# consensus-shipyard/ipc-filecoin-proofs

Measured on AMD Instinct MI355X. Metric: Merkle proofs verified/sec + HBM GB/s, 1M-receipt synthetic tipset, 1/2/4/8 GPU, higher is better.
Workload: dtype u64; 1 GPU; BASELINE.json configs[2] (the 1M-receipt tipset the metric is quoted on): 1000000 receipts (Amtv0<Receipt> + one Amt<...; receipts_per_gpu=1000000, claims_per_gpu=1000000, witness_blocks_per_gpu=1288038, witness_bytes_per_gpu=439923915, scan_matches=1002, device=AMD Radeon Graphics

## Files before the change

ipc-filecoin-proofs_amd/csrc/common.h:

```cpp
#pragma once
#include <hip/hip_runtime.h>

#include <cstdint>
#include <cstdio>
#include <memory>
#include <cstring>
#include <string>
#include <utility>
#include <vector>

#include "ipcfp.h"
#include "kernels/event_table.h"

namespace ipcfp {

struct DevPool {
    std::vector<std::pair<void*, size_t>> free_;
    size_t cached_bytes = 0;
    hipError_t take(void** out, size_t bytes, size_t* cap);
    void give(void* p, size_t cap);
    void drain();
    ~DevPool() { drain(); }
};
extern thread_local DevPool* g_tls_pool;
// ... 20 lines not shown
#endif
#ifndef IPCFP_PARSE_RESIDENT_DEFAULT
#define IPCFP_PARSE_RESIDENT_DEFAULT 1
#endif

struct ipcfp_ctx {
    int device = -1;
    hipStream_t stream = nullptr;
    hipStream_t stream_k1 = nullptr;
    hipStream_t stream_aux = nullptr;
    ipcfp::ScanParams scan_hint{};
    bool has_scan_hint = false;
    hipEvent_t aux_event = nullptr;
    std::string last_error;
    hipDeviceProp_t props{};
    ipcfp::DevPool pool;
    bool profiling = false;
    int profile_only = -1;
    std::vector<ipcfp::ProfiledLaunch> launches;
    std::vector<hipEvent_t> free_events;
    uint64_t prof_count[IPCFP_K_COUNT] = {};
    double prof_ms[IPCFP_K_COUNT] = {};
    uint8_t* pinned = nullptr;
    size_t pinned_cap = 0, pinned_used = 0;
    struct PendingRead {
        void* dst;
        size_t off, n;
        hipStream_t stream;
        bool hold = false;
    };
    std::vector<PendingRead> pending;
    int call_depth = 0;
    uint8_t* ctl_dev = nullptr;
    uint8_t* ctl_host = nullptr;
    uint32_t ctl_used_zero = 0, ctl_used_ff = 0;
    bool ctl_primed = false;
    bool ctl_preprimed = false;
    struct CtlRead {
        void* dst;
        uint32_t off, n;
    };
    std::vector<CtlRead> ctl_reads;
    hipEvent_t join_event = nullptr;
    hipEvent_t spin_event = nullptr;
    bool spin_sync = true;
    ipcfp::UploadRing* upload_ring = nullptr;
    hipStream_t stream_copy = nullptr;
    ipcfp::UploadTask* upload_task = nullptr;
    struct ClaimsExpand {
        bool pending = false;
        const void* compact_d = nullptr;
        const ipcfp_event_claim_group_t* groups_d = nullptr;
        uint32_t n = 0, n_groups = 0;
        const uint8_t* cblob_d = nullptr;
        uint64_t cblob_len = 0, cap_blob = 0;
        void* claims_out_d = nullptr;
        uint8_t* blob_out_d = nullptr;
        uint32_t* scratch_u32 = nullptr;
        uint64_t* scan_scratch = nullptr;
    } claims_expand;
    struct ClaimsRebase {
        bool pending = false;
        void* claims_d = nullptr;
        uint32_t n = 0;
        uint64_t base = 0, blob_len = 0;
        uint64_t full_len = 0;
// ... 23 lines not shown
    void* hamt_etabs = nullptr;
    size_t hamt_etabs_bytes = 0;
};

namespace ipcfp {

int set_error(ipcfp_ctx* ctx, int rc, const char* fmt, ...);

#define IPCFP_HIP(ctx, call)                                                                    \
    do {                                                                                        \
        hipError_t _e = (call);                                                                 \
        if (_e != hipSuccess)                                                                   \
            return ::ipcfp::set_error((ctx), IPCFP_E_HIP, "%s failed: %s (%s:%d)", #call,       \
                                      hipGetErrorString(_e), __FILE__, __LINE__);               \
    } while (0)

constexpr uint32_t kCtlHalf = 2048;

inline void* ctl_take(ipcfp_ctx* ctx, uint32_t bytes, bool ff) {
    if (!ctx->ctl_dev) return nullptr;
    bytes = (bytes + 7u) & ~7u;
    uint32_t& used = ff ? ctx->ctl_used_ff : ctx->ctl_used_zero;
    if (used + bytes > kCtlHalf) return nullptr;
    if (!ctx->ctl_primed) {
        if (hipMemcpyAsync(ctx->ctl_dev, ctx->ctl_host, 2 * kCtlHalf, hipMemcpyHostToDevice, ctx->stream) != hipSuccess) return nullptr;
        ctx->ctl_primed = true;
    }
    void* p = ctx->ctl_dev + (ff ? kCtlHalf : 0u) + used;
    used += bytes;
    ctx->ctl_preprimed = false;
    return p;
}
inline void ctl_preprime(ipcfp_ctx* ctx) {
    if (!ctx->ctl_dev || ctx->ctl_preprimed || ctx->call_depth != 1) return;
    if (hipMemcpyAsync(ctx->ctl_dev, ctx->ctl_host, 2 * kCtlHalf, hipMemcpyHostToDevice, ctx->stream) == hipSuccess) {
        ctx->ctl_preprimed = true;
    }
}
inline hipError_t ctl_fetch(ipcfp_ctx* ctx) {
    if (!ctx->ctl_dev || !ctx->ctl_primed) return hipSuccess;
    return hipMemcpyAsync(ctx->ctl_host + 2 * kCtlHalf, ctx->ctl_dev, 2 * kCtlHalf, hipMemcpyDeviceToHost, ctx->stream);
}
inline bool ctl_owns(const ipcfp_ctx* ctx, const void* dev_ptr) {
    const uint8_t* p = static_cast<const uint8_t*>(dev_ptr);
    return ctx->ctl_dev && p >= ctx->ctl_dev && p < ctx->ctl_dev + 2 * kCtlHalf;
}
template <typename T>
inline T ctl_value(const ipcfp_ctx* ctx, const void* dev_ptr) {
    T v;
    std::memcpy(&v, ctx->ctl_host + 2 * kCtlHalf + (static_cast<const uint8_t*>(dev_ptr) - ctx->ctl_dev), sizeof(T));
    return v;
}

inline hipError_t d2h_small(ipcfp_ctx* ctx, void* dst, const void* src_d, size_t n, hipStream_t s) {
    const size_t need = (n + 15) & ~size_t(15);
    if (!ctx->pinned || ctx->pinned_used + need > ctx->pinned_cap) return hipMemcpyAsync(dst, src_d, n, hipMemcpyDeviceToHost, s);
    const size_t off = ctx->pinned_used;
    ctx->pinned_used += need;
    ctx->pending.push_back({dst, off, n, s, false});
    return hipMemcpyAsync(ctx->pinned + off, src_d, n, hipMemcpyDeviceToHost, s);
}
inline hipError_t h2d_small(ipcfp_ctx* ctx, void* dst_d, const void* src, size_t n, hipStream_t s) {
    const size_t need = (n + 15) & ~size_t(15);
    if (!ctx->pinned || ctx->pinned_used + need > ctx->pinned_cap) return hipMemcpyAsync(dst_d, src, n, hipMemcpyHostToDevice, s);
    const size_t off = ctx->pinned_used;
    ctx->pinned_used += need;
    std::memcpy(ctx->pinned + off, src, n);
    ctx->pending.push_back({nullptr, off, 0, s, true});
    return hipMemcpyAsync(dst_d, ctx->pinned + off, n, hipMemcpyHostToDevice, s);
}
hipError_t wait_stream(ipcfp_ctx* ctx, hipStream_t s);

inline hipError_t sync_stream(ipcfp_ctx* ctx, hipStream_t s, bool last_of_call = false) {
    const bool ctl = s == ctx->stream && !ctx->ctl_reads.empty();
    if (ctl) (void)ctl_fetch(ctx);
    if (last_of_call && s == ctx->stream && ctx->ctl_dev && ctx->ctl_primed && !ctx->ctl_preprimed && ctx->call_depth == 1 &&
        hipMemcpyAsync(ctx->ctl_dev, ctx->ctl_host, 2 * kCtlHalf, hipMemcpyHostToDevice, ctx->stream) == hipSuccess) {
        ctx->ctl_preprimed = true;
    }
    const hipError_t e = wait_stream(ctx, s);
    if (ctl) {
        if (e == hipSuccess)
            for (auto& r : ctx->ctl_reads) std::memcpy(r.dst, ctx->ctl_host + 2 * kCtlHalf + r.off, r.n);
        ctx->ctl_reads.clear();
    }
    bool others = false;
    for (auto& r : ctx->pending) {
        if (r.stream == s) {
            if (r.dst && e == hipSuccess) std::memcpy(r.dst, ctx->pinned + r.off, r.n);
            r.dst = nullptr;
            r.hold = false;
        } else if (r.dst || r.hold) {
            others = true;
        }
    }
    if (!others) {
        ctx->pending.clear();
        ctx->pinned_used = 0;
    }
    return e;
}

int upload(ipcfp_ctx* ctx, void* dst_d, const void* src, size_t bytes, hipStream_t s);
bool upload_ring_mode();
UploadTask* upload_task_start(ipcfp_ctx* ctx, void* dst0, const void* src0, size_t bytes0, void* dst1, const void* src1, size_t bytes1);
int upload_task_wait(ipcfp_ctx* ctx);
int claims_ready(ipcfp_ctx* ctx);

struct ProfileScope {
// ... 58 lines not shown
        std::swap(p, o.p);
        std::swap(count, o.count);
        std::swap(cap, o.cap);
        std::swap(owner, o.owner);
    }
};

template <typename T>
inline hipError_t ctl_words(ipcfp_ctx* ctx, DevBuf<T>& own, T*& p, size_t count, bool ff) {
    p = static_cast<T*>(ctl_take(ctx, uint32_t(count * sizeof(T)), ff));
    if (p) return hipSuccess;
    hipError_t e = own.alloc(count);
    if (e != hipSuccess) return e;
    p = own.p;
    return hipMemsetAsync(own.p, ff ? 0xff : 0, count * sizeof(T), ctx->stream);
}
inline hipError_t ctl_read(ipcfp_ctx* ctx, void* dst, const void* p, size_t n) {
    if (ctl_owns(ctx, p)) {
        ctx->ctl_reads.push_back({dst, uint32_t(static_cast<const uint8_t*>(p) - ctx->ctl_dev), uint32_t(n)});
        return hipSuccess;
    }
    return d2h_small(ctx, dst, p, n, ctx->stream);
}

struct CallScope {
    DevPool* prev;
    ipcfp_ctx* ctx;
    explicit CallScope(ipcfp_ctx* c) : prev(g_tls_pool), ctx(c) {
        g_tls_pool = &c->pool;
        if (c->call_depth++ == 0) {
            c->pending.clear();
            c->pinned_used = 0;
            c->ctl_used_zero = c->ctl_used_ff = 0;
            c->ctl_primed = c->ctl_preprimed;
            c->ctl_reads.clear();
        }
    }
    ~CallScope() {
        g_tls_pool = prev;
        --ctx->call_depth;
    }
};
#define IPCFP_ENTER(ctx)                                 \
    IPCFP_HIP((ctx), hipSetDevice((ctx)->device));       \
    ::ipcfp::CallScope _ipcfp_call_scope(ctx)

inline uint32_t div_up(uint64_t a, uint64_t b) { return uint32_t((a + b - 1) / b); }

}

namespace ipcfp {
struct EnumCached {
    uint64_t root[5];
    int version = 0, vkind = 0;
    DevBuf<uint8_t> leaves;
    uint64_t n = 0;
    uint64_t error = ~0ULL;
    bool dense = false;
    uint64_t lo = 0, hi = ~0ULL;
};
struct EventTableCached {
    uint64_t root[5];
    uint64_t lo = 0, hi = ~0ULL;
    DevBuf<ReceiptRec> receipts;
    const EventRec* events = nullptr;
    uint64_t n = 0;
// ... 41 lines not shown
```

ipc-filecoin-proofs_amd/csrc/host/context.cpp:

```cpp
#include <algorithm>
#include <chrono>
#include <cstdarg>
#include <cstdlib>
#include <cstring>
#include <vector>

#include "../common.h"

namespace ipcfp {

int set_error(ipcfp_ctx* ctx, int rc, const char* fmt, ...) {
    char buf[512];
    va_list ap;
    va_start(ap, fmt);
    vsnprintf(buf, sizeof buf, fmt, ap);
    va_end(ap);
    if (ctx) ctx->last_error = buf;
    return rc;
}

thread_local DevPool* g_tls_pool = nullptr;

hipError_t wait_stream(ipcfp_ctx* ctx, hipStream_t s) {
    if (!ctx->spin_sync || !ctx->spin_event) return hipStreamSynchronize(s);
// ... 143 lines not shown
            ctx->stream_aux = ctx->stream;
        if (hipEventCreateWithFlags(&ctx->aux_event, hipEventDisableTiming) != hipSuccess) {
            if (ctx->stream_aux != ctx->stream) (void)hipStreamDestroy(ctx->stream_aux);
            ctx->stream_aux = ctx->stream;
            ctx->aux_event = nullptr;
        }
    }
    if (const char* e = std::getenv("IPCFP_SPIN_SYNC")) ctx->spin_sync = std::atoi(e) != 0;
    if (hipEventCreateWithFlags(&ctx->spin_event, hipEventDisableTiming) != hipSuccess) ctx->spin_event = nullptr;
    if (hipHostMalloc(reinterpret_cast<void**>(&ctx->pinned), 64 * 1024, hipHostMallocDefault) == hipSuccess)
        ctx->pinned_cap = 64 * 1024;
    else
        ctx->pinned = nullptr;
    {
        const char* e = std::getenv("IPCFP_MAILBOX");
        void* hp = nullptr;
        void* dp = nullptr;
        if (!(e && std::atoi(e) == 0) &&
            hipHostMalloc(&hp, 4096, hipHostMallocMapped | hipHostMallocCoherent) == hipSuccess) {
            if (hipHostGetDevicePointer(&dp, hp, 0) == hipSuccess &&
                hipEventCreateWithFlags(&ctx->main_event, hipEventDisableTiming) == hipSuccess) {
                if (hipEventCreateWithFlags(&ctx->rehash_event, hipEventDisableTiming) != hipSuccess) ctx->rehash_event = nullptr;
                std::memset(hp, 0, 4096);
                ctx->mailbox = static_cast<unsigned long long*>(hp);
                ctx->mailbox_dev = static_cast<unsigned long long*>(dp);
            } else {
                (void)hipHostFree(hp);
            }
        }
    }
    const char* ctl_env = std::getenv("IPCFP_CTL_BLOCK");
    if (!(ctl_env && std::atoi(ctl_env) == 0) &&
        hipHostMalloc(reinterpret_cast<void**>(&ctx->ctl_host), 4 * kCtlHalf, hipHostMallocDefault) == hipSuccess) {
        if (hipMalloc(reinterpret_cast<void**>(&ctx->ctl_dev), 2 * kCtlHalf) == hipSuccess) {
            std::memset(ctx->ctl_host, 0, kCtlHalf);
            std::memset(ctx->ctl_host + kCtlHalf, 0xff, kCtlHalf);
        } else {
            (void)hipHostFree(ctx->ctl_host);
            ctx->ctl_host = nullptr;
            ctx->ctl_dev = nullptr;
        }
    }
    *out = ctx;
    return IPCFP_OK;
}

void ipcfp_ctx_destroy(ipcfp_ctx_t* ctx) {
    if (!ctx) return;
    (void)hipSetDevice(ctx->device);
    (void)upload_task_wait(ctx);
    (void)hipStreamSynchronize(ctx->stream);
    (void)hipStreamSynchronize(ctx->stream_k1);
    (void)hipStreamSynchronize(ctx->stream_aux);
    if (ctx->scan_scratch) (void)hipFree(ctx->scan_scratch);
    if (ctx->hamt_recs) (void)hipFree(ctx->hamt_recs);
    if (ctx->hamt_scratch) (void)hipFree(ctx->hamt_scratch);
    if (ctx->hamt_etabs) (void)hipFree(ctx->hamt_etabs);
    for (auto& l : ctx->launches) {
        (void)hipEventDestroy(l.start);
        (void)hipEventDestroy(l.stop);
    }
    for (auto e : ctx->free_events) (void)hipEventDestroy(e);
    ctx->pool.drain();
    if (ctx->pinned) (void)hipHostFree(ctx->pinned);
    if (ctx->ctl_host) (void)hipHostFree(ctx->ctl_host);
    if (ctx->ctl_dev) (void)hipFree(ctx->ctl_dev);
    if (ctx->upload_ring) upload_ring_destroy(ctx->upload_ring);
    if (ctx->mailbox) (void)hipHostFree(ctx->mailbox);
    if (ctx->main_event) (void)hipEventDestroy(ctx->main_event);
    if (ctx->join_event) (void)hipEventDestroy(ctx->join_event);
    if (ctx->spin_event) (void)hipEventDestroy(ctx->spin_event);
    if (ctx->aux_event) (void)hipEventDestroy(ctx->aux_event);
    if (ctx->outline_event) (void)hipEventDestroy(ctx->outline_event);
    if (ctx->stream_aux != ctx->stream) (void)hipStreamDestroy(ctx->stream_aux);
    if (ctx->stream_k1 != ctx->stream) (void)hipStreamDestroy(ctx->stream_k1);
    if (ctx->rehash_event) (void)hipEventDestroy(ctx->rehash_event);
    if (ctx->stream_copy) (void)hipStreamDestroy(ctx->stream_copy);
    (void)hipStreamDestroy(ctx->stream);
    delete ctx;
}

const char* ipcfp_last_error(const ipcfp_ctx_t* ctx) { return ctx ? ctx->last_error.c_str() : "null context"; }

void* ipcfp_ctx_stream(ipcfp_ctx_t* ctx) { return ctx ? reinterpret_cast<void*>(ctx->stream) : nullptr; }

int ipcfp_ctx_set_tuning(ipcfp_ctx_t* ctx, const char* key, int64_t value) {
    if (!ctx || !key) return IPCFP_E_INVALID;
    const std::string k(key);
    if (k == "hamt_levels") ctx->hamt_levels = int(value);
    else if (k == "hamt_table") ctx->hamt_table = int(value);
    else if (k == "hamt_coop") ctx->hamt_coop = int(value);
    else if (k == "fast_verify") ctx->fast_verify = int(value);
    else if (k == "k1_resident" || k == "parse_resident") {
        if (value < 0 || value > int64_t(kResidentMax))
            return set_error(ctx, IPCFP_E_INVALID, "tuning key '%s': %lld is outside 0..%u", key, (long long)value, kResidentMax);
        (k == "k1_resident" ? ctx->k1_resident : ctx->parse_resident) = int(value);
    }
    else return set_error(ctx, IPCFP_E_INVALID, "unknown tuning key '%s'", key);
    return IPCFP_OK;
// ... 55 lines not shown
```

ipc-filecoin-proofs_amd/csrc/host/verify_events.cpp:

```cpp
#include <algorithm>
#include <cstring>
#include <memory>
#include <string>
#include <unordered_map>
#include <vector>

#include "../common.h"
#include "../kernels/claims_dev.h"
#include "../kernels/amt_enum.h"
#include "../kernels/event_table.h"
#include "../kernels/tipset_ctx.h"
#include "../kernels/types_dev.h"
#include "../kernels/launch.h"
#include "cidstr.h"
#include "exec_state.h"
#include "tipset_wide.h"
#include "pack_claims.h"

using namespace ipcfp;

namespace ipcfp {

void parse_cid_claim(const char* s, CidKey& key, bool& parsed, bool& canonical);
CidKey key_from_slot(const uint8_t* slot40);
// ... 177 lines not shown
            if (!have) {
                rc = enum_cache_put(ctx, w, tc.receipts_root, 0, VK_RECEIPT, w->receipt_lo, w->receipt_hi, *rec_en[k]);
                if (rc) return rc;
            }
        }
        const EnumCached* rc_enum = nullptr;
        rc = amt_enumerate_cached(ctx, w, tc.receipts_root, 0, VK_RECEIPT, &rc_enum, w->receipt_lo, w->receipt_hi);
        if (rc) return rc;
        if (rc_enum->error == kNoEnumError && rc_enum->dense) {
            tc.receipt_leaves = reinterpret_cast<const LeafRef*>(rc_enum->leaves.p);
            tc.n_receipt_leaves = rc_enum->n;
            tc.receipt_first = rc_enum->n ? w->receipt_lo : 0;
            if (w->use_event_table && rc_enum->n) {
                const EventTableCached* table = nullptr;
                rc = event_table_get(ctx, w, tc.receipts_root, rc_enum, &table);
                if (rc) return rc;
                tc.receipt_recs = table->receipts.p;
                tc.event_recs = table->events;
            }
        }
    }
    IPCFP_HIP(ctx, h2d_small(ctx, tcs_d.p, tcs.data(), tcs.size() * sizeof(TipsetCtxDev), ctx->stream));
    for (size_t k = 0; k < tcs.size(); ++k)
        if (tcs[k].exec_slots && execs[k]->status == IPCFP_ST_TRUE && execs[k]->total.p) {
            rc = launch_exec_finish(ctx, tcs_d.p + k, execs[k]->total.p, execs[k]->first.p, execs[k]->pos.p,
                                    uint32_t(execs[k]->raw_len), execs[k]->inv.p);
            if (rc) return rc;
        }
    rc = event_table_join(ctx, w);
    if (rc) return rc;
    bool tabulated = false;
    for (auto& tc : tcs) tabulated = tabulated || tc.receipt_recs != nullptr;
    if ((rc = claims_ready(ctx))) return rc;
    rc = launch_verify_events(ctx, view, claims_d, n, tcs_d.p, uint32_t(tcs.size()), blob_d, blob_len,
                              trust ? *trust : accept_all, filter, status_d, where_d, tabulated);
    if (rc) return rc;
    IPCFP_HIP(ctx, sync_stream(ctx, ctx->stream));
    return IPCFP_OK;
}

}


extern "C" {

static int verify_event_proofs_impl(ipcfp_ctx_t* ctx, ipcfp_witness_t* w, const ipcfp_event_proof_t* proofs, uint64_t n,
                                    const ipcfp_trust_policy_t* trust, const ipcfp_event_filter_t* filter,
                                    ipcfp_status_t* status, ipcfp_value_loc_t* event_loc);

int ipcfp_verify_event_proofs(ipcfp_ctx_t* ctx, ipcfp_witness_t* w, const ipcfp_event_proof_t* proofs, uint64_t n,
                              const ipcfp_trust_policy_t* trust, const ipcfp_event_filter_t* filter,
                              ipcfp_status_t* status) {
    return verify_event_proofs_impl(ctx, w, proofs, n, trust, filter, status, nullptr);
}

int ipcfp_verify_event_proofs_located(ipcfp_ctx_t* ctx, ipcfp_witness_t* w, const ipcfp_event_proof_t* proofs, uint64_t n,
                                      const ipcfp_trust_policy_t* trust, const ipcfp_event_filter_t* filter,
                                      ipcfp_status_t* status, ipcfp_value_loc_t* event_loc) {
    if (n && !event_loc) return IPCFP_E_INVALID;
    return verify_event_proofs_impl(ctx, w, proofs, n, trust, filter, status, event_loc);
}

int ipcfp_verify_event_proofs_with(ipcfp_ctx_t* ctx, ipcfp_witness_t* w, const ipcfp_event_proof_t* proofs, uint64_t n,
                                   const ipcfp_trust_policy_t* trust, const ipcfp_event_filter_t* filter,
                                   ipcfp_check_event_fn check_event, void* user, ipcfp_status_t* status) {
    if (!check_event) return verify_event_proofs_impl(ctx, w, proofs, n, trust, filter, status, nullptr);
    if (n == 0) return ctx && w && w->ctx == ctx ? IPCFP_OK : IPCFP_E_INVALID;
    std::vector<ipcfp_value_loc_t> loc(n);
// ... 360 lines not shown
```

ipc-filecoin-proofs_amd/csrc/host/verify_fast.cpp:

```cpp
#include <chrono>
#include <cstring>
#include <memory>
#include <vector>

#include "../common.h"
#include "../kernels/claims_dev.h"
#include "../kernels/amt_enum.h"
#include "../kernels/event_table.h"
#include "../kernels/tipset_ctx.h"
#include "../kernels/types_dev.h"
#include "../kernels/launch.h"
#include "exec_state.h"

using namespace ipcfp;

namespace ipcfp {

int exec_state_prepare(ipcfp_ctx* ctx, ExecState& ex, uint32_t n_parents);

static int verify_packed_fast_queue(ipcfp_ctx* ctx, ipcfp_witness* w, std::vector<TipsetCtxDev>& tcs, const EventClaimPacked* claims_d,
                                    uint32_t n, const uint8_t* blob_d, uint64_t blob_len, const ipcfp_trust_policy_t* trust,
                                    const ipcfp_event_filter_t* filter, uint8_t* status_d, void* where_d, bool* done, ScanRide* ride);

int verify_packed_fast(ipcfp_ctx* ctx, ipcfp_witness* w, std::vector<TipsetCtxDev>& tcs, const EventClaimPacked* claims_d,
// ... 159 lines not shown
                                    ride_offsets.p, ride->cap_matches ? ride->matches_d : nullptr, ride->matches_d ? ride->cap_matches : 0,
                                    ride->has_d, ride->has_d ? n_rcpt : 0, w->receipt_lo, tail_scratch, ++ctx->scan_epoch, table_err,
                                    err_p, ctx->mailbox_dev, ride_seq);
        if (rc) return rc;
        ctx->scan_hint = want;
        ctx->has_scan_hint = true;
    }
    if (defer_rehash) {
        rc = launch_txmeta_rehash(ctx, ctx->stream_aux, view, tcs_d.p, ex.err.p);
        if (rc) return rc;
    }
    prof.reset(new ProfileScope(ctx, IPCFP_K_EXEC_ORDER));
    rc = launch_exec_insert_flags(ctx, ex.keys.p, n_msgs, ex.slots.p, ex.mask, ex.first.p);
    if (rc) return rc;
    IPCFP_HIP(ctx, ctl_words(ctx, ex.total_own, ex.total.p, 1, false));
    CtxFinish fin{};
    fin.err = ex.err.p;
    fin.total = ex.total.p;
    fin.first = ex.first.p;
    fin.pos = ex.pos.p;
    fin.inv = ex.inv.p;
    fin.slots = ex.slots.p;
    fin.keys = ex.keys.p;
    fin.mask = ex.mask;
    fin.raw_len = n_msgs;
    fin.receipt_leaves = rleaves.p;
    fin.n_receipt_leaves = n_rcpt;
    fin.receipt_first = w->receipt_lo;
    fin.receipt_recs = table->receipts.p;
    fin.event_recs = table->events;
    rc = launch_exec_scan_finish(ctx, tcs_d.p, fin, ex.pos.p, ex.total.p, scan_ctl);
    if (rc) return rc;
    prof.reset();
    rc = event_table_join(ctx, w);
    if (rc) return rc;
    if ((rc = claims_ready(ctx))) return rc;
    rc = launch_verify_events(ctx, view, claims_d, n, tcs_d.p, 1, blob_d, blob_len, trust ? *trust : accept_all, filter, status_d,
                              where_d, true);
    if (rc) return rc;
    if (defer_rehash || ride_seq) {
        hipEvent_t aux_done = defer_rehash ? ctx->rehash_event : ctx->aux_event;
        IPCFP_HIP(ctx, hipEventRecord(aux_done, ctx->stream_aux));
        IPCFP_HIP(ctx, hipStreamWaitEvent(ctx->stream, aux_done, 0));
    }
    uint32_t bad = 0;
    unsigned long long e = kNoEnumError;
    TipsetCtxDev facts;
    IPCFP_HIP(ctx, ctl_read(ctx, &bad, small + 2, 4));
    IPCFP_HIP(ctx, ctl_read(ctx, &e, ex.err.p, 8));
    IPCFP_HIP(ctx, ctl_read(ctx, &facts, tcs_d.p, sizeof facts));
    IPCFP_HIP(ctx, sync_stream(ctx, ctx->stream, true));
    IPCFP_HIP(ctx, hipGetLastError());
    if (bad || e != kNoEnumError || facts.child_status != IPCFP_ST_TRUE) {
        IPCFP_HIP(ctx, hipStreamSynchronize(ctx->stream_aux));
        w->bt_joined = true;
        return IPCFP_OK;
    }
    tcs[0] = facts;
    {
        std::unique_ptr<EnumCached> en(new EnumCached());
        std::memcpy(en->root, facts.receipts_root.w, 40);
        en->version = 0;
        en->vkind = VK_RECEIPT;
        en->lo = w->receipt_lo;
        en->hi = w->receipt_hi;
        en->n = n_rcpt;
        en->error = kNoEnumError;
        en->dense = true;
        en->leaves.p = reinterpret_cast<uint8_t*>(rleaves.p);
        en->leaves.count = rleaves.count * sizeof(LeafRef);
        en->leaves.cap = rleaves.cap;
// ... 31 lines not shown
```

ipc-filecoin-proofs_amd/csrc/kernels/launch.h:

```cpp
#pragma once
#include <cstdint>

#include "../common.h"
#include "witness_dev.h"

namespace ipcfp {

int launch_chunk_order(ipcfp_ctx* ctx, const uint32_t* len_d, uint32_t n, uint32_t* bins_d, uint32_t* order_d);
int launch_k1_layout(ipcfp_ctx* ctx, const uint32_t* len_d, uint32_t n, uint32_t* bins_d, uint32_t* order_d,
                     uint32_t* sched_len_d, uint64_t* sched_off_d, uint64_t* total_d, uint64_t* scan_scratch_d,
                     uint64_t* off_by_id_d, void* meta_d);
int launch_gather_cids(ipcfp_ctx* ctx, const uint32_t* order_d, const uint8_t* cids_d, uint32_t n, uint8_t* sched_cids_d);
int launch_blake2b256_cid(ipcfp_ctx* ctx, const uint8_t* arena, const void* meta, const uint8_t* sched_cids40, uint32_t n,
                          uint32_t* ok_bits, uint8_t* status, unsigned long long* counters);
int launch_blake2b256_raw(ipcfp_ctx* ctx, const uint8_t* arena, const void* meta, uint32_t n, uint8_t* out32);

int launch_aligned_offsets(ipcfp_ctx* ctx, const uint32_t* len_d, uint32_t n, uint64_t* new_off_d,
                           uint64_t* total_d, uint64_t* scratch_d );
int launch_tight_offsets(ipcfp_ctx* ctx, const uint32_t* len_d, uint32_t n, uint64_t* off_d, uint64_t* total_d,
                         uint64_t* scratch_d );
int launch_expand_cids(ipcfp_ctx* ctx, const uint8_t* digests32_d, uint32_t n, const uint8_t* prefix, uint32_t prefix_len,
                       const uint32_t* esc_index_d, const uint8_t* esc_cids40_d, uint32_t n_esc, uint8_t* cids40_d);
int launch_repack(ipcfp_ctx* ctx, const uint8_t* src, const uint64_t* old_off, const uint32_t* len,
                  const uint64_t* new_off, uint32_t n, uint8_t* dst);
// ... 69 lines not shown
                    uint64_t* scratch_d);

struct TipsetCtxDev;
struct AmtRootSpec;
struct ReceiptRec;
struct EventRec;
struct EventTableView;
struct LeafRef;
struct EventClaimPacked;
int launch_ctx_headers(ipcfp_ctx* ctx, const WitnessView& w, TipsetCtxDev* ctxs_d, uint32_t n);
struct CtxFinish;
int launch_ctx_finish(ipcfp_ctx* ctx, TipsetCtxDev* ctx_d, const CtxFinish& a);
int launch_exec_scan_finish(ipcfp_ctx* ctx, TipsetCtxDev* ctx_d, const CtxFinish& a, uint32_t* pos_d, uint64_t* total_d,
                            unsigned long long* ctl_d);
size_t exec_scan_ctl_words(uint32_t n);
int launch_exec_insert(ipcfp_ctx* ctx, const CidKey* keys_d, uint32_t n, unsigned long long* slots_d, uint32_t mask);
int launch_exec_insert_flags(ipcfp_ctx* ctx, const CidKey* keys_d, uint32_t n, unsigned long long* slots_d, uint32_t mask,
                             uint32_t* first_d);
int launch_exec_finish(ipcfp_ctx* ctx, TipsetCtxDev* ctx_d, const uint64_t* total_d, const uint32_t* first_d,
                       const uint32_t* pos_d, uint32_t n, uint32_t* inv_d);
int launch_tipset_prepare(ipcfp_ctx* ctx, const WitnessView& w, const void* jobs, const void* jobs_d, uint32_t n_jobs,
                          bool need_general, bool defer_rehash = false,
                          const void* inline_inputs = nullptr);
int launch_exec_roots(ipcfp_ctx* ctx, const WitnessView& w, const TipsetCtxDev* ctx_d, AmtRootSpec* roots_d,
                      unsigned long long* err_d, int verify_txmeta = 1, uint32_t n_parents = 0);
int launch_tipset_prepare_wide(ipcfp_ctx* ctx, const WitnessView& w, const void* job, uint32_t n_parents);
int launch_exec_dedup(ipcfp_ctx* ctx, const WitnessView& w, const LeafRef* leaves_d, uint32_t n, CidKey* keys_d,
                      unsigned long long* slots_d, uint32_t mask, uint32_t* first_d);
int launch_exec_compact(ipcfp_ctx* ctx, const CidKey* keys_d, uint32_t n, const uint32_t* first_d,
                        const uint32_t* pos_d, CidKey* out_d);
int launch_verify_events(ipcfp_ctx* ctx, const WitnessView& w, const EventClaimPacked* claims_d, uint32_t n,
                         const TipsetCtxDev* ctxs_d, uint32_t n_ctxs, const uint8_t* blob_d, uint64_t blob_len,
                         const ipcfp_trust_policy_t& trust, const ipcfp_event_filter_t* filter, uint8_t* status_d,
                         void* where_d = nullptr, bool tabulated = false);
int launch_verify_events_table(ipcfp_ctx* ctx, const WitnessView& w, const EventClaimPacked* claims_d, uint32_t n,
                               const TipsetCtxDev* ctxs_d, uint32_t n_ctxs, const uint8_t* blob_d, uint64_t blob_len,
                               const ipcfp_trust_policy_t& trust, const ipcfp_event_filter_t& filter, int has_filter,
                               uint8_t* status_d, void* where_d);

int launch_scan_pass1(ipcfp_ctx* ctx, const WitnessView& w, const LeafRef* receipts_d, uint32_t n,
                      const ipcfp_event_filter_t& filter, int has_actor, uint64_t actor, uint32_t* counts_d,
                      unsigned long long* err_d);
int launch_scan_pass2(ipcfp_ctx* ctx, const WitnessView& w, const CidKey& receipts_root, const LeafRef* receipts_d,
                      uint32_t n, const ipcfp_event_filter_t& filter, int has_actor, uint64_t actor,
                      const uint32_t* counts_d, const uint32_t* offsets_d, void* matches_d, uint64_t matches_cap,
                      uint8_t* has_match_d, uint64_t has_cap, uint64_t has_base = 0,
                      const EventTableView* table = nullptr);
struct BlockRec;
int launch_receipt_walk(ipcfp_ctx* ctx, const WitnessView& w, const LeafRef* receipts_d, uint32_t n,
                        const ipcfp_event_filter_t* filter, int has_actor, uint64_t actor, const ReceiptRec* rrecs_d,
                        uint32_t* counts_d, unsigned long long* err_d, hipStream_t stream);
int launch_receipt_events(ipcfp_ctx* ctx, const WitnessView& w, const LeafRef* receipts_d, uint32_t n,
                          const ipcfp_event_filter_t* filter, int has_actor, uint64_t actor, const BlockRec* brecs_d,
                          ReceiptRec* rrecs_d, uint32_t* counts_d, unsigned long long* err_d, hipStream_t stream = nullptr);
int launch_block_events(ipcfp_ctx* ctx, hipStream_t stream, const uint8_t* arena, const void* meta_d, uint32_t n,
                        const ipcfp_event_filter_t* filter, int has_actor, uint64_t actor, BlockRec* brecs_d,
                        EventRec* erecs_d, uint32_t cap_events, uint32_t* pool_used_d);
int launch_scan_tail_fused(ipcfp_ctx* ctx, const WitnessView& w, const LeafRef* receipts_d, uint32_t n, uint64_t dense_first,
                           const ipcfp_event_filter_t& filter, int has_actor, uint64_t actor, const EventTableView& table,
                           const uint32_t* counts_d, uint32_t* offsets_d, void* matches_d, uint64_t matches_cap, uint8_t* has_match_d,
                           uint64_t has_cap, uint64_t has_base, unsigned long long* scratch_d, unsigned long long epoch,
                           const unsigned long long* err_a_d, const unsigned long long* err_b_d, unsigned long long* mailbox_dev,
                           unsigned long long seq);
int launch_count_from_table(ipcfp_ctx* ctx, const WitnessView& w, const LeafRef* receipts_d, uint32_t n,
                            const ipcfp_event_filter_t& filter, int has_actor, uint64_t actor, const EventTableView& table,
                            uint32_t* counts_d, unsigned long long* err_d);

int launch_base64_decode(ipcfp_ctx* ctx, const uint8_t* text_d, const void* spans_d, uint32_t n_blocks, uint32_t n_units,
                         const uint64_t* dst_off_d, uint8_t* arena_d, unsigned long long* first_bad_d);

int launch_parse_cid_arrays(ipcfp_ctx* ctx, const uint8_t* text_d, const void* spans_d, uint32_t n, uint8_t* cids_d,
// ... 52 lines not shown
```

ipc-filecoin-proofs_amd/csrc/kernels/verify_events.hip:

```cpp
#define IPCFP_LINE_STAGE 1
#include <hip/hip_runtime.h>

#include "../common.h"
#include "blake2b_dev.h"
#include "claims_dev.h"
#include "event_log_dev.h"
#include "walk_dev.h"
#include "amt_enum.h"
#include "event_table.h"
#include "tipset_ctx.h"
#include "types_dev.h"
#include "launch.h"
#include "scan_dev.h"
#include "verify_dev.h"

namespace ipcfp {

__global__ __launch_bounds__(256) void k_exec_keys(WitnessView w, const LeafRef* __restrict__ leaves, uint32_t n,
                                                   CidKey* __restrict__ keys) {
    const uint32_t t = blockIdx.x * blockDim.x + threadIdx.x;
    if (t >= n) return;
    const LeafRef l = leaves[t];
    Rd r;
    r.init(w.arena + w.off[l.block] + l.off, l.len);
// ... 225 lines not shown
    if (rr.at_null()) return IPCFP_ST_FALSE_NO_EVENTS_ROOT;
    CidKey events_root;
    rr.read_link_key(events_root);
    ValueLoc eloc;
    st = amt_load_get(w, events_root, 3, VK_STAMPED_EVENT, c.event_index, eloc);
    if (st == IPCFP_ST_NOT_FOUND) return IPCFP_ST_FALSE_NO_EVENT;
    if (st != IPCFP_ST_TRUE) return st;
    if (where) *where = eloc;
    Rd er;
    er.init(w.arena + w.off[eloc.block] + eloc.off, eloc.len);
    uint64_t emitter;
    EvmLogLoc log;
    decode_event_log(er, emitter, log);
    if (emitter != c.emitter) return IPCFP_ST_FALSE_EMITTER;
    if (!log.is_log) return IPCFP_ST_FALSE_NOT_EVM_LOG;
    if (log.n_topics != c.n_topics) return IPCFP_ST_FALSE_TOPIC_COUNT;
    for (uint32_t i = 0; i < log.n_topics; ++i) {
        const uint8_t* claimed = blob + c.topics_off + 33u * i;
        if (!claimed[0]) return IPCFP_ST_FALSE_TOPIC;
        if (!er.equal32(log.topic_at(i), claimed + 1)) return IPCFP_ST_FALSE_TOPIC;
    }
    if (!(c.flags & EC_DATA_MATCHABLE) || c.data_len != log.data.len) return IPCFP_ST_FALSE_DATA;
    if (!er.equal_bytes(log.data.off, blob + c.data_off, c.data_len)) return IPCFP_ST_FALSE_DATA;
    if (has_filter && !log_matches(er, log, filter)) return IPCFP_ST_FALSE_FILTER;
    return IPCFP_ST_TRUE;
}

__global__ __launch_bounds__(256, IPCFP_WALK_WAVES) void k_verify_events(WitnessView w, const EventClaimPacked* __restrict__ claims,
                                                       uint32_t n, const TipsetCtxDev* __restrict__ ctxs, uint32_t n_ctxs,
                                                       const uint8_t* __restrict__ blob, uint64_t blob_len,
                                                       ipcfp_trust_policy_t trust,
                                                       ipcfp_event_filter_t filter, int has_filter,
                                                       uint8_t* __restrict__ status, ValueLoc* __restrict__ where,
                                                       int pending_only) {
    const uint32_t t = blockIdx.x * blockDim.x + threadIdx.x;
    if (t >= n) return;
    if (pending_only && status[t] != kStPending) return;
    const EventClaimPacked& c = claims[t];
    ValueLoc loc{kNoBlock, 0, 0};
    uint32_t st = IPCFP_ST_ERR_BAD_CLAIM;
    if (claim_in_bounds(c, n_ctxs, blob_len))
        st = verify_event_one(w, c, ctxs[c.context], blob, trust, filter, has_filter != 0, where ? &loc : nullptr);
    status[t] = uint8_t(st);
    if (where) where[t] = loc;
}

__global__ __launch_bounds__(256) void k_exec_finish(TipsetCtxDev* __restrict__ c, const uint64_t* __restrict__ total,
                                                     const uint32_t* __restrict__ first, const uint32_t* __restrict__ pos,
                                                     uint32_t n, uint32_t* __restrict__ inv) {
    const uint32_t i = blockIdx.x * blockDim.x + threadIdx.x;
    if (i == 0) c->exec_len = *total;
    if (i < n && first[i]) inv[pos[i]] = i;
}

__global__ __launch_bounds__(256) void k_ctx_finish(TipsetCtxDev* __restrict__ c, CtxFinish a) {
    const uint32_t i = blockIdx.x * blockDim.x + threadIdx.x;
    if (i < a.raw_len && a.first[i]) a.inv[a.pos[i]] = i;
    if (i == 0) ctx_finish_fields(c, a, *a.total);
}

int launch_exec_scan_finish(ipcfp_ctx* ctx, TipsetCtxDev* ctx_d, const CtxFinish& a, uint32_t* pos_d, uint64_t* total_d,
                            unsigned long long* ctl_d) {
    const uint32_t n = a.raw_len;
    if (n == 0) return set_error(ctx, IPCFP_E_INVALID, "exec scan: no messages");
    hipLaunchKernelGGL(k_exec_scan_finish, dim3(div_up(n, kExecTile)), dim3(256), 0, ctx->stream, a.first, n, pos_d, total_d, ctl_d,
                       ctx_d, a);
    IPCFP_HIP(ctx, hipGetLastError());
// ... 23 lines not shown
    hipLaunchKernelGGL(k_exec_insert, g, b, 0, ctx->stream, keys_d, n, slots_d, mask);
    hipLaunchKernelGGL(k_exec_first, g, b, 0, ctx->stream, keys_d, n, slots_d, mask, first_d);
    IPCFP_HIP(ctx, hipGetLastError());
    return IPCFP_OK;
}

int launch_exec_insert(ipcfp_ctx* ctx, const CidKey* keys_d, uint32_t n, unsigned long long* slots_d, uint32_t mask) {
    if (n == 0) return IPCFP_OK;
    hipLaunchKernelGGL(k_exec_insert, dim3(div_up(n, 256)), dim3(256), 0, ctx->stream, keys_d, n, slots_d, mask);
    IPCFP_HIP(ctx, hipGetLastError());
    return IPCFP_OK;
}

int launch_exec_insert_flags(ipcfp_ctx* ctx, const CidKey* keys_d, uint32_t n, unsigned long long* slots_d, uint32_t mask,
                             uint32_t* first_d) {
    if (n == 0) return IPCFP_OK;
    hipLaunchKernelGGL(k_exec_insert_flags, dim3(div_up(n, 256)), dim3(256), 0, ctx->stream, keys_d, n, slots_d, mask, first_d);
    IPCFP_HIP(ctx, hipGetLastError());
    return IPCFP_OK;
}

int launch_exec_compact(ipcfp_ctx* ctx, const CidKey* keys_d, uint32_t n, const uint32_t* first_d,
                        const uint32_t* pos_d, CidKey* out_d) {
    if (n == 0) return IPCFP_OK;
    hipLaunchKernelGGL(k_exec_compact, dim3(div_up(n, 256)), dim3(256), 0, ctx->stream, keys_d, n, first_d, pos_d,
                       out_d);
    IPCFP_HIP(ctx, hipGetLastError());
    return IPCFP_OK;
}

int launch_verify_events(ipcfp_ctx* ctx, const WitnessView& w, const EventClaimPacked* claims_d, uint32_t n,
                         const TipsetCtxDev* ctxs_d, uint32_t n_ctxs, const uint8_t* blob_d, uint64_t blob_len,
                         const ipcfp_trust_policy_t& trust, const ipcfp_event_filter_t* filter, uint8_t* status_d,
                         void* where_d, bool tabulated) {
    if (n == 0) return IPCFP_OK;
    ipcfp_event_filter_t f{};
    if (filter) f = *filter;
    {
        ProfileScope prof(ctx, IPCFP_K_EVENT_VERIFY);
        if (tabulated) {
            int rc = launch_verify_events_table(ctx, w, claims_d, n, ctxs_d, n_ctxs, blob_d, blob_len, trust, f, filter ? 1 : 0,
                                                status_d, where_d);
            if (rc) return rc;
        }
        hipLaunchKernelGGL(k_verify_events, dim3(div_up(n, 256)), dim3(256), 0, ctx->stream, w, claims_d, n, ctxs_d,
                           n_ctxs, blob_d, blob_len, trust, f, filter ? 1 : 0, status_d, static_cast<ValueLoc*>(where_d),
                           tabulated ? 1 : 0);
    }
    IPCFP_HIP(ctx, hipGetLastError());
    return IPCFP_OK;
}

}
```

ipc-filecoin-proofs_amd/csrc/kernels/verify_table.hip:

```cpp
#include <hip/hip_runtime.h>

#include "../common.h"
#include "launch.h"
#include "verify_dev.h"

namespace ipcfp {

typedef unsigned long long u64x2_t __attribute__((ext_vector_type(2)));

__device__ __forceinline__ u64x2_t ld16(const uint8_t* __restrict__ p) {
    u64x2_t v;
    __builtin_memcpy(&v, p, 16);
    return v;
}
__device__ __forceinline__ bool differ32(const u64x2_t a[2], const u64x2_t b[2]) {
    return (((a[0].x ^ b[0].x) | (a[0].y ^ b[0].y)) | ((a[1].x ^ b[1].x) | (a[1].y ^ b[1].y))) != 0;
}

struct ClaimedBytes {
    u64x2_t topic[2][2];
    uint32_t flag[2];
    u64x2_t data[2];
};

// ... 53 lines not shown
        __builtin_memcpy(f0, filter.topic0, 32);
        __builtin_memcpy(f1, filter.topic1, 32);
        if (differ32(t0, f0) || differ32(t1, f1)) return IPCFP_ST_FALSE_FILTER;
    }
    return IPCFP_ST_TRUE;
}

__device__ __forceinline__ uint32_t verify_table_one(const WitnessView& w, const EventClaimPacked& c, const TipsetCtxDev& tc,
                                                     const uint8_t* __restrict__ blob, const ipcfp_trust_policy_t& trust,
                                                     const ipcfp_event_filter_t& filter, bool has_filter, ValueLoc* where) {
    ClaimedBytes p;
    load_claimed(c, blob, p);
    const bool tabulated = tc.receipt_leaves && tc.receipt_recs && c.exec_index >= tc.receipt_first &&
                           c.exec_index - tc.receipt_first < tc.n_receipt_leaves;
    ReceiptRec rr{RK_WALK, 0, 0, kNoBlock, 0};
    if (tabulated) rr = tc.receipt_recs[c.exec_index - tc.receipt_first];
    const uint32_t st = verify_event_prefix(c, tc, trust);
    if (st != IPCFP_ST_TRUE) return st;
    if (!tabulated || rr.kind == RK_WALK) return kStPending;
    if (rr.kind == RK_NO_EVENTS) return IPCFP_ST_FALSE_NO_EVENTS_ROOT;
    if (rr.kind >= 64) return rr.kind;
    if (c.event_index == ~0ULL) return IPCFP_ST_ERR;
    if (c.event_index >= 64 || !((rr.bitmap >> c.event_index) & 1ull)) return IPCFP_ST_FALSE_NO_EVENT;
    const EventRec e = tc.event_recs[rr.first + __popcll(rr.bitmap & ((1ull << c.event_index) - 1ull))];
    if (where) *where = ValueLoc{rr.block, uint32_t((e.base_flags & kEvBaseMask) - w.off[rr.block]), e.ev_len};
    return verify_event_record_batched(w, c, e, p, blob, filter, has_filter);
}

__global__ __launch_bounds__(256) void k_verify_events_table(WitnessView w, const EventClaimPacked* __restrict__ claims, uint32_t n,
                                                             const TipsetCtxDev* __restrict__ ctxs, uint32_t n_ctxs,
                                                             const uint8_t* __restrict__ blob, uint64_t blob_len,
                                                             ipcfp_trust_policy_t trust, ipcfp_event_filter_t filter,
                                                             int has_filter, uint8_t* __restrict__ status,
                                                             ValueLoc* __restrict__ where) {
    const uint32_t t = blockIdx.x * blockDim.x + threadIdx.x;
    const bool live = t < n;
    EventClaimPacked c;
    if (live) c = claims[t];
    else c.context = 0;
    ValueLoc loc{kNoBlock, 0, 0};
    uint32_t st = IPCFP_ST_ERR_BAD_CLAIM;
    const bool inb = live && claim_in_bounds(c, n_ctxs, blob_len);
    const uint32_t ctx0 = __builtin_amdgcn_readfirstlane(inb ? c.context : 0xffffffffu);
    if (__all(!inb || c.context == ctx0)) {
        if (inb) st = verify_table_one(w, c, ctxs[ctx0], blob, trust, filter, has_filter != 0, where ? &loc : nullptr);
    } else if (inb) {
        st = verify_table_one(w, c, ctxs[c.context], blob, trust, filter, has_filter != 0, where ? &loc : nullptr);
    }
    if (!live) return;
    status[t] = uint8_t(st);
    if (where) where[t] = loc;
}

int launch_verify_events_table(ipcfp_ctx* ctx, const WitnessView& w, const EventClaimPacked* claims_d, uint32_t n,
                               const TipsetCtxDev* ctxs_d, uint32_t n_ctxs, const uint8_t* blob_d, uint64_t blob_len,
                               const ipcfp_trust_policy_t& trust, const ipcfp_event_filter_t& filter, int has_filter,
                               uint8_t* status_d, void* where_d) {
    if (n == 0) return IPCFP_OK;
    hipLaunchKernelGGL(k_verify_events_table, dim3(div_up(n, 256)), dim3(256), 0, ctx->stream, w, claims_d, n, ctxs_d, n_ctxs,
                       blob_d, blob_len, trust, filter, has_filter, status_d, static_cast<ValueLoc*>(where_d));
    IPCFP_HIP(ctx, hipGetLastError());
    return IPCFP_OK;
}

}
```

Before: 1.245 billion proofs/s.

## Skip pending-event fallback kernel when table pass leaves nothing pending; double-buffer control block

The table-driven event verify kernel now counts claims it leaves pending, using a wave ballot plus one atomic per wave into a zeroed control word. The fallback walk kernel reads that count and exits at once when it is zero, so the full-grid status scan is skipped in the common case. The device control block is also doubled, and a spare half is primed before the next call and swapped in at call entry, so the reset copy can overlap earlier work. This adds an atomic per wave and more state for tracking which control buffer is primed.

```diff
diff --git a/ipc-filecoin-proofs_amd/csrc/common.h b/ipc-filecoin-proofs_amd/csrc/common.h
--- a/ipc-filecoin-proofs_amd/csrc/common.h
+++ b/ipc-filecoin-proofs_amd/csrc/common.h
@@ -76,6 +76,9 @@
     std::vector<PendingRead> pending;
     int call_depth = 0;
     uint8_t* ctl_dev = nullptr;
+    uint8_t* ctl_alt = nullptr;
+    uint8_t* ctl_alloc = nullptr;
+    bool ctl_alt_primed = false;
     uint8_t* ctl_host = nullptr;
     uint32_t ctl_used_zero = 0, ctl_used_ff = 0;
     bool ctl_primed = false;
@@ -165,10 +168,15 @@
     return p;
 }
 inline void ctl_preprime(ipcfp_ctx* ctx) {
-    if (!ctx->ctl_dev || ctx->ctl_preprimed || ctx->call_depth != 1) return;
+    if (!ctx->ctl_dev || ctx->ctl_preprimed || ctx->ctl_alt_primed || ctx->call_depth != 1) return;
     if (hipMemcpyAsync(ctx->ctl_dev, ctx->ctl_host, 2 * kCtlHalf, hipMemcpyHostToDevice, ctx->stream) == hipSuccess) {
         ctx->ctl_preprimed = true;
     }
+}
+inline void ctl_prime_alt(ipcfp_ctx* ctx) {
+    if (!ctx->ctl_alt || ctx->ctl_alt_primed || ctx->call_depth != 1) return;
+    if (hipMemcpyAsync(ctx->ctl_alt, ctx->ctl_host, 2 * kCtlHalf, hipMemcpyHostToDevice, ctx->stream) == hipSuccess)
+        ctx->ctl_alt_primed = true;
 }
 inline hipError_t ctl_fetch(ipcfp_ctx* ctx) {
     if (!ctx->ctl_dev || !ctx->ctl_primed) return hipSuccess;
@@ -207,7 +215,8 @@
 inline hipError_t sync_stream(ipcfp_ctx* ctx, hipStream_t s, bool last_of_call = false) {
     const bool ctl = s == ctx->stream && !ctx->ctl_reads.empty();
     if (ctl) (void)ctl_fetch(ctx);
-    if (last_of_call && s == ctx->stream && ctx->ctl_dev && ctx->ctl_primed && !ctx->ctl_preprimed && ctx->call_depth == 1 &&
+    if (last_of_call && s == ctx->stream && ctx->ctl_dev && ctx->ctl_primed && !ctx->ctl_preprimed && !ctx->ctl_alt_primed &&
+        ctx->call_depth == 1 &&
         hipMemcpyAsync(ctx->ctl_dev, ctx->ctl_host, 2 * kCtlHalf, hipMemcpyHostToDevice, ctx->stream) == hipSuccess) {
         ctx->ctl_preprimed = true;
     }
@@ -332,6 +341,11 @@
             c->pending.clear();
             c->pinned_used = 0;
             c->ctl_used_zero = c->ctl_used_ff = 0;
+            if (!c->ctl_preprimed && c->ctl_alt_primed) {
+                std::swap(c->ctl_dev, c->ctl_alt);
+                c->ctl_preprimed = true;
+                c->ctl_alt_primed = false;
+            }
             c->ctl_primed = c->ctl_preprimed;
             c->ctl_reads.clear();
         }
diff --git a/ipc-filecoin-proofs_amd/csrc/host/context.cpp b/ipc-filecoin-proofs_amd/csrc/host/context.cpp
--- a/ipc-filecoin-proofs_amd/csrc/host/context.cpp
+++ b/ipc-filecoin-proofs_amd/csrc/host/context.cpp
@@ -199,7 +199,9 @@
     const char* ctl_env = std::getenv("IPCFP_CTL_BLOCK");
     if (!(ctl_env && std::atoi(ctl_env) == 0) &&
         hipHostMalloc(reinterpret_cast<void**>(&ctx->ctl_host), 4 * kCtlHalf, hipHostMallocDefault) == hipSuccess) {
-        if (hipMalloc(reinterpret_cast<void**>(&ctx->ctl_dev), 2 * kCtlHalf) == hipSuccess) {
+        if (hipMalloc(reinterpret_cast<void**>(&ctx->ctl_alloc), 4 * kCtlHalf) == hipSuccess) {
+            ctx->ctl_dev = ctx->ctl_alloc;
+            ctx->ctl_alt = ctx->ctl_alloc + 2 * kCtlHalf;
             std::memset(ctx->ctl_host, 0, kCtlHalf);
             std::memset(ctx->ctl_host + kCtlHalf, 0xff, kCtlHalf);
         } else {
@@ -231,7 +233,7 @@
     ctx->pool.drain();
     if (ctx->pinned) (void)hipHostFree(ctx->pinned);
     if (ctx->ctl_host) (void)hipHostFree(ctx->ctl_host);
-    if (ctx->ctl_dev) (void)hipFree(ctx->ctl_dev);
+    if (ctx->ctl_alloc) (void)hipFree(ctx->ctl_alloc);
     if (ctx->upload_ring) upload_ring_destroy(ctx->upload_ring);
     if (ctx->mailbox) (void)hipHostFree(ctx->mailbox);
     if (ctx->main_event) (void)hipEventDestroy(ctx->main_event);
diff --git a/ipc-filecoin-proofs_amd/csrc/host/verify_events.cpp b/ipc-filecoin-proofs_amd/csrc/host/verify_events.cpp
--- a/ipc-filecoin-proofs_amd/csrc/host/verify_events.cpp
+++ b/ipc-filecoin-proofs_amd/csrc/host/verify_events.cpp
@@ -233,8 +233,11 @@
     bool tabulated = false;
     for (auto& tc : tcs) tabulated = tabulated || tc.receipt_recs != nullptr;
     if ((rc = claims_ready(ctx))) return rc;
+    DevBuf<uint32_t> pending_own;
+    uint32_t* pending_d = nullptr;
+    if (tabulated) IPCFP_HIP(ctx, ctl_words(ctx, pending_own, pending_d, 2, false));
     rc = launch_verify_events(ctx, view, claims_d, n, tcs_d.p, uint32_t(tcs.size()), blob_d, blob_len,
-                              trust ? *trust : accept_all, filter, status_d, where_d, tabulated);
+                              trust ? *trust : accept_all, filter, status_d, where_d, tabulated, pending_d);
     if (rc) return rc;
     IPCFP_HIP(ctx, sync_stream(ctx, ctx->stream));
     return IPCFP_OK;
diff --git a/ipc-filecoin-proofs_amd/csrc/host/verify_fast.cpp b/ipc-filecoin-proofs_amd/csrc/host/verify_fast.cpp
--- a/ipc-filecoin-proofs_amd/csrc/host/verify_fast.cpp
+++ b/ipc-filecoin-proofs_amd/csrc/host/verify_fast.cpp
@@ -215,11 +215,15 @@
     rc = launch_exec_scan_finish(ctx, tcs_d.p, fin, ex.pos.p, ex.total.p, scan_ctl);
     if (rc) return rc;
     prof.reset();
+    DevBuf<uint32_t> pending_own;
+    uint32_t* pending_d = nullptr;
+    IPCFP_HIP(ctx, ctl_words(ctx, pending_own, pending_d, 2, false));
+    ctl_prime_alt(ctx);
     rc = event_table_join(ctx, w);
     if (rc) return rc;
     if ((rc = claims_ready(ctx))) return rc;
     rc = launch_verify_events(ctx, view, claims_d, n, tcs_d.p, 1, blob_d, blob_len, trust ? *trust : accept_all, filter, status_d,
-                              where_d, true);
+                              where_d, true, pending_d);
     if (rc) return rc;
     if (defer_rehash || ride_seq) {
         hipEvent_t aux_done = defer_rehash ? ctx->rehash_event : ctx->aux_event;
diff --git a/ipc-filecoin-proofs_amd/csrc/kernels/launch.h b/ipc-filecoin-proofs_amd/csrc/kernels/launch.h
--- a/ipc-filecoin-proofs_amd/csrc/kernels/launch.h
+++ b/ipc-filecoin-proofs_amd/csrc/kernels/launch.h
@@ -125,11 +125,11 @@
 int launch_verify_events(ipcfp_ctx* ctx, const WitnessView& w, const EventClaimPacked* claims_d, uint32_t n,
                          const TipsetCtxDev* ctxs_d, uint32_t n_ctxs, const uint8_t* blob_d, uint64_t blob_len,
                          const ipcfp_trust_policy_t& trust, const ipcfp_event_filter_t* filter, uint8_t* status_d,
-                         void* where_d = nullptr, bool tabulated = false);
+                         void* where_d = nullptr, bool tabulated = false, uint32_t* pending_d = nullptr);
 int launch_verify_events_table(ipcfp_ctx* ctx, const WitnessView& w, const EventClaimPacked* claims_d, uint32_t n,
                                const TipsetCtxDev* ctxs_d, uint32_t n_ctxs, const uint8_t* blob_d, uint64_t blob_len,
                                const ipcfp_trust_policy_t& trust, const ipcfp_event_filter_t& filter, int has_filter,
-                               uint8_t* status_d, void* where_d);
+                               uint8_t* status_d, void* where_d, uint32_t* pending_d = nullptr);
 
 int launch_scan_pass1(ipcfp_ctx* ctx, const WitnessView& w, const LeafRef* receipts_d, uint32_t n,
                       const ipcfp_event_filter_t& filter, int has_actor, uint64_t actor, uint32_t* counts_d,
diff --git a/ipc-filecoin-proofs_amd/csrc/kernels/verify_events.hip b/ipc-filecoin-proofs_amd/csrc/kernels/verify_events.hip
--- a/ipc-filecoin-proofs_amd/csrc/kernels/verify_events.hip
+++ b/ipc-filecoin-proofs_amd/csrc/kernels/verify_events.hip
@@ -281,7 +281,8 @@
                                                        ipcfp_trust_policy_t trust,
                                                        ipcfp_event_filter_t filter, int has_filter,
                                                        uint8_t* __restrict__ status, ValueLoc* __restrict__ where,
-                                                       int pending_only) {
+                                                       int pending_only, const uint32_t* __restrict__ n_pending) {
+    if (n_pending && *n_pending == 0) return;
     const uint32_t t = blockIdx.x * blockDim.x + threadIdx.x;
     if (t >= n) return;
     if (pending_only && status[t] != kStPending) return;
@@ -371,7 +372,7 @@
 int launch_verify_events(ipcfp_ctx* ctx, const WitnessView& w, const EventClaimPacked* claims_d, uint32_t n,
                          const TipsetCtxDev* ctxs_d, uint32_t n_ctxs, const uint8_t* blob_d, uint64_t blob_len,
                          const ipcfp_trust_policy_t& trust, const ipcfp_event_filter_t* filter, uint8_t* status_d,
-                         void* where_d, bool tabulated) {
+                         void* where_d, bool tabulated, uint32_t* pending_d) {
     if (n == 0) return IPCFP_OK;
     ipcfp_event_filter_t f{};
     if (filter) f = *filter;
@@ -379,15 +380,15 @@
         ProfileScope prof(ctx, IPCFP_K_EVENT_VERIFY);
         if (tabulated) {
             int rc = launch_verify_events_table(ctx, w, claims_d, n, ctxs_d, n_ctxs, blob_d, blob_len, trust, f, filter ? 1 : 0,
-                                                status_d, where_d);
+                                                status_d, where_d, pending_d);
             if (rc) return rc;
         }
         hipLaunchKernelGGL(k_verify_events, dim3(div_up(n, 256)), dim3(256), 0, ctx->stream, w, claims_d, n, ctxs_d,
                            n_ctxs, blob_d, blob_len, trust, f, filter ? 1 : 0, status_d, static_cast<ValueLoc*>(where_d),
-                           tabulated ? 1 : 0);
-    }
-    IPCFP_HIP(ctx, hipGetLastError());
-    return IPCFP_OK;
-}
-
-}
+                           tabulated ? 1 : 0, tabulated ? static_cast<const uint32_t*>(pending_d) : nullptr);
+    }
+    IPCFP_HIP(ctx, hipGetLastError());
+    return IPCFP_OK;
+}
+
+}
diff --git a/ipc-filecoin-proofs_amd/csrc/kernels/verify_table.hip b/ipc-filecoin-proofs_amd/csrc/kernels/verify_table.hip
--- a/ipc-filecoin-proofs_amd/csrc/kernels/verify_table.hip
+++ b/ipc-filecoin-proofs_amd/csrc/kernels/verify_table.hip
@@ -109,7 +109,7 @@
                                                              const uint8_t* __restrict__ blob, uint64_t blob_len,
                                                              ipcfp_trust_policy_t trust, ipcfp_event_filter_t filter,
                                                              int has_filter, uint8_t* __restrict__ status,
-                                                             ValueLoc* __restrict__ where) {
+                                                             ValueLoc* __restrict__ where, uint32_t* __restrict__ pending) {
     const uint32_t t = blockIdx.x * blockDim.x + threadIdx.x;
     const bool live = t < n;
     EventClaimPacked c;
@@ -124,6 +124,10 @@
     } else if (inb) {
         st = verify_table_one(w, c, ctxs[c.context], blob, trust, filter, has_filter != 0, where ? &loc : nullptr);
     }
+    if (pending) {
+        const unsigned long long left = __ballot(live && st == kStPending);
+        if (left && (threadIdx.x & 63u) == 0) atomicAdd(pending, uint32_t(__popcll(left)));
+    }
     if (!live) return;
     status[t] = uint8_t(st);
     if (where) where[t] = loc;
@@ -132,10 +136,10 @@
 int launch_verify_events_table(ipcfp_ctx* ctx, const WitnessView& w, const EventClaimPacked* claims_d, uint32_t n,
                                const TipsetCtxDev* ctxs_d, uint32_t n_ctxs, const uint8_t* blob_d, uint64_t blob_len,
                                const ipcfp_trust_policy_t& trust, const ipcfp_event_filter_t& filter, int has_filter,
-                               uint8_t* status_d, void* where_d) {
+                               uint8_t* status_d, void* where_d, uint32_t* pending_d) {
     if (n == 0) return IPCFP_OK;
     hipLaunchKernelGGL(k_verify_events_table, dim3(div_up(n, 256)), dim3(256), 0, ctx->stream, w, claims_d, n, ctxs_d, n_ctxs,
-                       blob_d, blob_len, trust, filter, has_filter, status_d, static_cast<ValueLoc*>(where_d));
+                       blob_d, blob_len, trust, filter, has_filter, status_d, static_cast<ValueLoc*>(where_d), pending_d);
     IPCFP_HIP(ctx, hipGetLastError());
     return IPCFP_OK;
 }
```

Result: slower. 1.215 billion proofs/s (-2.5%).
